# WD-Leong/CV-Lite-Object-Detection

Measured on AMD Instinct MI355X. Metric: training images/sec (whole node), FCOS-VOC 512x512 bs=16/GPU, higher is better.
Workload: dtype bf16; 1 GPU; FCOS ResNet-50-FPN train step (targets + fwd + loss + bwd + clip/SGD), 512x512, bs=16 per GPU; model=FCOS-ResNet50-FPN, global_batch=16, image_size=512, parallelism=dp1

## Files before the change

cv-lite-object-detection_amd/csrc/conv_common.h:

```cpp
#pragma once
#include "cvl_common.h"
#include "bn_acc.h"
#include <type_traits>
#include <vector>

typedef short s16x8 __attribute__((ext_vector_type(8)));
typedef short s16x4 __attribute__((ext_vector_type(4)));
typedef __bf16 bf16x8 __attribute__((ext_vector_type(8)));
typedef float f32x4 __attribute__((ext_vector_type(4)));

constexpr int kMaxSeg = CVL_CONV_MAX_SEG;

extern thread_local int g_cvl_conv_last_kernel;
extern thread_local int g_cvl_conv_last_ktile;

__device__ __forceinline__ int xcd_remap(int b, int nwg) {
  const int q = nwg / 8, r = nwg % 8, x = b % 8;
  return (x < r ? x * (q + 1) : r * (q + 1) + (x - r) * q) + b / 8;
}

template <int N>
__device__ __forceinline__ void wait_vm() {
  __builtin_amdgcn_s_waitcnt((N & 15) | ((N >> 4) << 14) | (7 << 4) | (15 << 8));
}

__device__ __forceinline__ s16x4 ds_tr16(unsigned addr) {
  s16x4 v;
  asm volatile("ds_read_b64_tr_b16 %0, %1" : "=v"(v) : "v"(addr));
  return v;
}
__device__ __forceinline__ void lgkm_wait() { asm volatile("s_waitcnt lgkmcnt(0)" ::: "memory"); }
__device__ __forceinline__ void tr_pin(s16x4& v) { asm volatile("" : "+v"(v)); }
__device__ __forceinline__ s16x8 tr_join(s16x4 l, s16x4 h) {
  return s16x8{l[0], l[1], l[2], l[3], h[0], h[1], h[2], h[3]};
}

__device__ __forceinline__ unsigned lds_addr(const void* p) {
  return (unsigned)(size_t)(const __attribute__((address_space(3))) void*)p;
}

struct ConvSeg {
  int Hr, Wr, Hs, Ws;
  long src_base, src_img, dst_base, dst_img;
  int m_start;
  int rows;
  const cvl_bf16* w;
  const float* bias;
// ... 51 lines not shown
int cvl_wgrad_reduce(const float* slab, float* dst0, float* dst1, long n4, int splits, int groups, float beta,
                     hipStream_t s);
int cvl_wgrad_defer_guard(const float* dst, hipStream_t s);
int cvl_wgrad_reduce_lanes(long elems4, int splits);

struct BnSumArgs {
  const cvl_bf16* z;
  const float* mr;
  const float* gamma;
  const float* beta;
  acc_u64* sums;
  float hi;
  const cvl_bf16* y;
  const uint8_t* bits;
};

enum { CVL_BSUM_NONE = 0, CVL_BSUM_Z = 1, CVL_BSUM_Y = 2, CVL_BSUM_BITS = 3 };
struct ConvCallOpts {
  bool bn_stats;
  int bsum;
  bool ymask;
  size_t workspace_bytes;
};

enum { CVL_PRE_NONE = 0, CVL_PRE_ZERO_GAPS = 1, CVL_PRE_S2DG3_PACK = 2 };

struct ConvPlan {
  int kernel;
  int bn, bk;
  bool dgrad;
  bool sw;
  bool wres;
  bool prio, acc, stamps;
  int stages;
  int bsum;
  bool ymask;
  int splits, ksteps_per_split;
  int grid;
  size_t workspace_bytes;
  int pre;
  size_t pack_bytes;
  int dbg;
  cvl_conv_desc desc;
  ConvArgs geo;
};

int conv_plan(const cvl_conv_desc* d, const ConvCallOpts& o, ConvPlan* p);
size_t conv_plan_workspace_bound(const cvl_conv_desc* d);
static inline void conv_plan_set_splits(ConvPlan* p, int nk, int want) {
  p->ksteps_per_split = (nk + want - 1) / want;
  p->splits = (nk + p->ksteps_per_split - 1) / p->ksteps_per_split;
}
static inline int conv_plan_ktile(const ConvPlan& p) { return p.kernel == CVL_CK_X32 || p.kernel == CVL_CK_P ? p.bk : 0; }

int launch_base(const ConvPlan& p, const ConvArgs& a, hipStream_t s);
int launch_l(const ConvPlan& p, const ConvArgs& a, hipStream_t s);
int launch_x(const ConvPlan& p, const ConvArgs& a, hipStream_t s);
int launch_h(const ConvPlan& p, const ConvArgs& a, hipStream_t s);
int launch_p(const ConvPlan& p, const ConvArgs& a, hipStream_t s);

bool cvl_conv_h_fits(const cvl_conv_desc* d, const ConvArgs& a, int* halo_px);
constexpr int kConvHWresCb = 2;
constexpr int kConvHStampWgs = 4096;
constexpr unsigned kConvBufRecords = 0x7fffffffu;

template <class F>
// ... 137 lines not shown
```

cv-lite-object-detection_amd/csrc/conv_dispatch.hip:

```cpp
#include "conv_common.h"

namespace {

constexpr int BM_BASE = 128, NT_BASE = 256;
constexpr int BM = 256;
constexpr int H_BN = 64, H_BK = 32;

int device_cus() {
  static const int n = cvl_device_cus();
  return n;
}

int pick_bn(int npad) { return npad % 128 == 0 ? 128 : (npad % 64 == 0 ? 64 : 32); }

int base_split_want(const ConvArgs& a) {
  if (a.nseg != 1) return 1;
  const int BN_ = pick_bn(a.Npad), BK_ = a.Cin % 64 == 0 ? 64 : 32;
  const int tiles = a.m_tiles * (a.Npad / BN_);
  const int nk = a.K / BK_;
  const int max_tiles = cvl_tune_int("CVL_KSPLIT_MAX_TILES", 192);
  const int target = cvl_tune_int("CVL_KSPLIT_TARGET", 384);
  const int min_nk = cvl_dispatch_int("ksplit_min_nk", 4);
  if (tiles >= max_tiles || nk < min_nk) return 1;
  int s = (target + tiles - 1) / tiles;
// ... 111 lines not shown
                 (a.dst_up != 1 && !by) || o.bn_stats || (a.seg[0].Hr * a.seg[0].Wr) % BM ||
                 (a.dst_up == 1 && a.seg[0].dst_img != (long)a.seg[0].Hr * a.seg[0].Wr) || a.Npad % 64))
    return false;
  if (d->mode == CVL_CONV_DGRAD && d->stride != 1) return false;
  const ConvSeg& q = a.seg[0];
  if (d->stride == 1 && (q.Hs != q.Hr || q.Ws != q.Wr)) return false;
  if (a.dst_f32 ? (a.n_store % 4 || a.ld_dst % 4 || a.dst_coff % 4) : !dst_chunks8(d)) return false;
  if (o.bn_stats && (a.dst_f32 || (q.Hr * q.Wr) % BM)) return false;
  return buffer_bounds_ok(a);
}

bool plan_p(const cvl_conv_desc* d, const ConvArgs& a, const ConvCallOpts& o, ConvPlan* p) {
  if (cvl_dispatch_flag("no_p") || !p_fits(d, a, o)) return false;
  if (o.bsum && cvl_tune_flag("CVL_CONV_P_NO_BSUM")) return false;
  const bool wide = a.K <= 256 || (a.Npad >= 2 * a.K && cvl_dispatch_int("p_wide128", 1));
  const int bn = wide && a.Npad % 128 == 0 ? 128 : (a.Npad % 64 == 0 ? 64 : 0);
  const int fbn = cvl_dispatch_int("p_bn", 0);
  const int use = o.bsum ? 64 : (fbn && a.Npad % fbn == 0 ? fbn : bn);
  if (!use) return false;
  const int ntiles = a.m_tiles * (a.Npad / use);
  const int ntn = a.Npad / use;
  const int wgs = cvl_dispatch_int("p_wgs", 256);
  int grid = cvl_tune_int("CVL_CONV_P_WGS", wgs > 256 ? 256 : (wgs < 1 ? 1 : wgs));
  if (grid >= ntiles) grid = ntiles;
  else grid -= grid % ntn;
  if (grid < 1) return false;
  p->kernel = CVL_CK_P;
  p->bn = use;
  p->bk = a.K % 64 == 0 && use != 256 && cvl_dispatch_int("p_k64", 1) ? 64 : 32;
  p->grid = grid;
  p->dbg = cvl_tune_int("CVL_P_ABLATE", 0);
  p->bsum = o.bsum;
  p->acc = a.beta != 0.f && !cvl_tune_flag("CVL_P_NO_ACC");
  return true;
}

bool plan_h(const cvl_conv_desc* d, const ConvArgs& a, const ConvCallOpts& o, size_t ws_bytes, ConvPlan* p) {
  int halo_px = 0;
  if (cvl_dispatch_flag("no_h") || !cvl_conv_h_fits(d, a, &halo_px)) return false;
  const bool stg3 = !cvl_dispatch_flag("h_no_3stage") && halo_px <= 512;
  const bool bs = o.bsum != CVL_BSUM_NONE;
  p->kernel = CVL_CK_H64;
  p->bk = H_BK;
  p->bsum = o.bsum;
  if (a.Npad == 32) {
    if (o.bn_stats || bs) return false;
    p->bn = 32;
    p->stages = stg3 ? 3 : 2;
    p->grid = a.m_tiles < device_cus() ? a.m_tiles : device_cus();
    return true;
  }
  const int tiles = a.m_tiles * (a.Npad / H_BN);
  const bool sw_ok = !d->dst_f32 && d->beta == 0.f && dst_chunks8(d) && !(o.bn_stats && bs) && tiles_in_images(a, bs);
  if (!cvl_dispatch_flag("h_no_n32") && a.Npad % H_BN == 0 && 2 * tiles <= device_cus() && sw_ok) {
    p->bn = 32;
    p->sw = true;
    p->stages = stg3 ? 3 : 2;
    p->grid = 2 * tiles;
    return true;
  }
  const int ncb = a.Cin / H_BK;
  int splits = 1;
  if (a.nseg == 1 && !bs && ws_bytes && d->n_store % 8 == 0 && d->dst_coff % 8 == 0 &&
      (d->dst_f32 || d->ld_dst % 8 == 0) && d->n_store / 8 <= 256) {
    splits = h_split_want(a);
    if (slab_bytes(a, splits) > ws_bytes) splits = 1;
// ... 205 lines not shown
```

cv-lite-object-detection_amd/csrc/conv_igemm.hip:

```cpp
#include "conv_common.h"

namespace {

constexpr int BM = 128;
constexpr int NT = 256;

template <int BK>
__device__ __forceinline__ int swz(int r) {
  return BK == 128 ? (r & 15) : (BK == 64 ? ((r >> 1) & 7) : ((r >> 2) & 3));
}

__device__ __forceinline__ s16x8 relu_bf16x8(s16x8 v) {
#pragma unroll
  for (int i = 0; i < 8; ++i) v[i] = v[i] < 0 ? (short)0 : v[i];
  return v;
}



template <int BN, int BK, bool DGRAD>
__global__ void __launch_bounds__(NT) conv_igemm_kernel(ConvArgs a) {
  constexpr int WM = BM / 2, WN = BN / 2;
  constexpr int TM = WM / 16, TN = WN / 16;
  constexpr int CPR = BK / 8;
// ... 438 lines not shown
  const void* ymask;
  void* workspace;
};

void fill_args(const ConvPlan& p, const ConvIo& io, ConvArgs* a) {
  *a = p.geo;
  a->src = reinterpret_cast<const cvl_bf16*>(io.src);
  a->dst = io.dst;
  a->stats = io.stats;
  if (p.bsum) {
    const BnSumArgs& b = *io.bsum;
    a->bz = b.z; a->bmr = b.mr; a->bga = b.gamma; a->bbe = b.beta; a->bsum = b.sums; a->bhi = b.hi;
    a->by = b.y;
    a->bbits = b.bits;
  }
  if (p.ymask) a->ymask = reinterpret_cast<const cvl_bf16*>(io.ymask);
  if (p.kernel == CVL_CK_X32) a->probe = reinterpret_cast<unsigned long long*>(cvl_probe_current(true));
  a->dbg = p.dbg;
  a->splits = p.splits;
  a->ksteps_per_split = p.ksteps_per_split;
  char* ws = reinterpret_cast<char*>(io.workspace);
  if (p.splits > 1) a->slab = reinterpret_cast<float*>(ws + p.pack_bytes);
  if (p.pre == CVL_PRE_S2DG3_PACK)
    for (int i = 0; i < kMaxSeg; ++i)
      a->seg[i].w = reinterpret_cast<const cvl_bf16*>(ws) + (size_t)(i < a->nseg ? i : 0) * a->Npad * a->K;
}

}

thread_local int g_cvl_conv_last_kernel = CVL_CK_NONE;
thread_local int g_cvl_conv_last_ktile = 0;

extern "C" int cvl_conv_igemm_last_kernel(void) { return g_cvl_conv_last_kernel; }
extern "C" int cvl_conv_igemm_last_ktile(void) { return g_cvl_conv_last_ktile; }

int launch_base(const ConvPlan& p, const ConvArgs& a, hipStream_t s) {
  if (p.bn == 128) launch_bn<128>(p, a, s);
  else if (p.bn == 64) launch_bn<64>(p, a, s);
  else launch_bn<32>(p, a, s);
  return cvl_launch_status();
}

namespace {
int conv_run(const ConvPlan& p, const cvl_conv_desc* d, const ConvIo& io, hipStream_t s) {
  int st = pre_pass(p, d, io.dst, io.workspace, s);
  if (st) return st;
  ConvArgs a;
  fill_args(p, io, &a);
  switch (p.kernel) {
    case CVL_CK_P: st = launch_p(p, a, s); break;
    case CVL_CK_X32: st = launch_x(p, a, s); break;
    case CVL_CK_H64: st = launch_h(p, a, s); break;
    case CVL_CK_L64: case CVL_CK_L128: case CVL_CK_L256: st = launch_l(p, a, s); break;
    default: st = launch_base(p, a, s); break;
  }
  g_cvl_conv_last_kernel = p.kernel;
  g_cvl_conv_last_ktile = conv_plan_ktile(p);
  if (st || p.splits <= 1) return st;
  return splitk_finish_launch(a, s);
}
}

extern "C" const char* cvl_conv_kernel_name(int code) {
  switch (code) {
    case CVL_CK_BASE: return "conv_igemm_kernel (128-row)";
    case CVL_CK_BASE_SPLITK: return "conv_igemm_kernel (128-row, split-K)";
    case CVL_CK_L64: return "conv_igemm_l_kernel<64> (256x64)";
    case CVL_CK_L128: return "conv_igemm_l_kernel<128> (256x128)";
    case CVL_CK_L256: return "conv_igemm_l_kernel<256> (256x256)";
    case CVL_CK_X256: return "conv_igemm_x_kernel (256x256, 4 phases per 64-deep K-tile)";
    case CVL_CK_X32: return "conv_igemm_x32_kernel (256x256, 5-slot ring of 32-deep K-tiles)";
    case CVL_CK_X32H: return "conv_igemm_x32h_kernel (256x256, 3x3 halo tile in LDS, 6-slot weight ring)";
    case CVL_CK_WG_SN: return "conv_wgrad_sn_kernel (Npad 32, taps on the dY side, chunk slabs)";
    case CVL_CK_WG_S: return "conv_wgrad_kernel (128-wide k tile)";
    case CVL_CK_WG_L128: return "conv_wgrad_l_kernel<128> (128x256)";
    case CVL_CK_WG_L256: return "conv_wgrad_l_kernel<256> (256x256)";
    case CVL_CK_WG_X: return "conv_wgrad_x_kernel (256x256, 5-slot ring of 32-row steps, grouped)";
    case CVL_CK_WG_H: return "conv_wgrad_h_kernel (64 ci x 64 co x 9 taps, 128-row halo steps)";
    case CVL_CK_H64: return "conv_igemm_h_kernel (256x64, 3x3 halo + 9-tap weight stage per channel block)";
    case CVL_CK_P: return "conv_igemm_p_kernel (persistent 1x1, K-tile stream across tiles)";
    default: return "none";
  }
}

int cvl_conv_f32(const cvl_conv_desc* d, const void* src, void* dst, acc_u64* bn_stats, hipStream_t s);
int cvl_relu_backward(const void* dy, const void* y, void* dx, long n, float beta, cvl_stream_t stream);

extern "C" size_t cvl_conv_igemm_workspace_size(const cvl_conv_desc* d) {
  if (!d) return 0;
  if (d->prec == CVL_PREC_F32) return 16;
// ... 141 lines not shown
```

cv-lite-object-detection_amd/csrc/conv_igemm_p.hip:

```cpp
#include "conv_common.h"

namespace {

constexpr int NT = 512, BM = 256;
constexpr unsigned kRecords = 0x7fffffffu;
constexpr unsigned kOOB = 0x80000000u;
constexpr int LDS_BYTES = 163840;

template <int BK>
__device__ __forceinline__ int swz(int r) { return (r >> 1) & (BK / 8 - 1); }

__device__ __forceinline__ void dma16(__amdgpu_buffer_rsrc_t r, const void* lds_dst, unsigned voff) {
  __builtin_amdgcn_raw_ptr_buffer_load_lds(r, (__attribute__((address_space(3))) void*)lds_dst, 16, (int)voff, 0,
                                           0, 0);
}

template <int BN, int BK>
struct PCfg {
  static constexpr int WGM = BN == 256 ? 2 : 4, WGN = 8 / WGM;
  static constexpr int WM = BM / WGM, WN = BN / WGN, TM = WM / 16, TN = WN / 16;
  static constexpr int SLOT_B = (BM + BN) * BK * 2;
  static constexpr int PR = 8 * 64 * 16 / (BK * 2);
  static constexpr int APW = BM / PR;
  static constexpr int BPW = BN >= PR ? BN / PR : 1;
  static constexpr int PW = APW + BPW;
  static constexpr int RED_B = WGM * BN * 2 * 4;
  static constexpr int DUMMY_B = BN < PR ? 4 * 1024 : 0;
  static constexpr int NS = (LDS_BYTES - RED_B - DUMMY_B) / SLOT_B;
  static constexpr int D = NS - 1;
  static_assert(D >= 2, "ring too short");
};

typedef __bf16 bf16x2 __attribute__((ext_vector_type(2)));
typedef float f32x2 __attribute__((ext_vector_type(2)));
typedef unsigned u32x4 __attribute__((ext_vector_type(4)));

__device__ __forceinline__ void wait_vm_atleast(int n) {
  if (n >= 63) wait_vm<63>();
  else if (n >= 48) wait_vm<48>();
  else if (n >= 36) wait_vm<36>();
  else if (n >= 30) wait_vm<30>();
  else if (n >= 24) wait_vm<24>();
  else if (n >= 21) wait_vm<21>();
  else if (n >= 18) wait_vm<18>();
  else if (n >= 15) wait_vm<15>();
  else if (n >= 12) wait_vm<12>();
  else if (n >= 9) wait_vm<9>();
  else if (n >= 6) wait_vm<6>();
  else if (n >= 3) wait_vm<3>();
  else wait_vm<0>();
}

__device__ __forceinline__ s16x8 gload16_untracked(const void* p) {
  s16x8 v;
  asm volatile("global_load_dwordx4 %0, %1, off" : "=v"(v) : "v"(p) : "memory");
  return v;
}
__device__ __forceinline__ void pin16(s16x8& v) { asm volatile("" : "+v"(v)); }
__device__ __forceinline__ unsigned gload1_untracked(const void* p) {
  unsigned v;
  asm volatile("global_load_ubyte %0, %1, off" : "=v"(v) : "v"(p) : "memory");
  return v;
}
__device__ __forceinline__ void pin1(unsigned& v) { asm volatile("" : "+v"(v)); }

template <int BN, int BK, bool RELU, bool F32, int BS = 0, bool ACC = false>
__global__ void __launch_bounds__(NT) conv_igemm_p_kernel(ConvArgs a, int ntiles) {
  using C = PCfg<BN, BK>;
  constexpr int TM = C::TM, TN = C::TN, NS = C::NS, D = C::D;
  __shared__ __attribute__((aligned(16))) char lds[C::NS * C::SLOT_B + C::RED_B + C::DUMMY_B];
  float* red = reinterpret_cast<float*>(lds + NS * C::SLOT_B);
  char* dummy = lds + NS * C::SLOT_B + C::RED_B;

  const int tid = threadIdx.x;
  const int wave = __builtin_amdgcn_readfirstlane(tid >> 6), lane = tid & 63;
  const ConvSeg& S = a.seg[0];
  const int HWr = S.Hr * S.Wr;
  const int ntn = a.Npad / BN;
  const int nk = a.K / BK;
  const int G = gridDim.x;
  const int L = xcd_remap(blockIdx.x, G);
  const int nmc = G / ntn;
  const int mchunk = (a.m_tiles + nmc - 1) / nmc;
  const int mt0 = (L / ntn) * mchunk;
  const int my_tiles = max(0, min(mchunk, a.m_tiles - mt0));
  const int total = my_tiles * nk;
  const bool dense_src = a.stride == 1 && S.Hs == S.Hr && S.Ws == S.Wr && S.src_img == (long)HWr;
  const int Cin2 = a.Cin * 2;
  const int K2 = a.K * 2;

  constexpr int LPR = BK / 8, PR = C::PR, WR = PR / 8;
  const int prow = wave * WR + lane / LPR, ch = lane % LPR;
  const unsigned chs = (unsigned)((ch ^ swz<BK>(prow)) * 16);
  const __amdgpu_buffer_rsrc_t rsA = __builtin_amdgcn_make_buffer_rsrc((void*)a.src, (short)0, (int)kRecords, 0x00020000);
  const __amdgpu_buffer_rsrc_t rsB = __builtin_amdgcn_make_buffer_rsrc((void*)S.w, (short)0, (int)kRecords, 0x00020000);

  int ik = 0, it = 0, islot = 0;
  unsigned ia[C::APW], ib[C::BPW];
  const int n0 = (L % ntn) * BN;
  auto set_issue_tile = [&](int k) {
    const int m0 = (mt0 + k) * BM;
#pragma unroll
    for (int p = 0; p < C::APW; ++p) {
// ... 56 lines not shown
  for (int i = 0; i < TM; ++i)
#pragma unroll
    for (int j = 0; j < TN; ++j) acc[i][j] = f32x4{0.f, 0.f, 0.f, 0.f};

  float bcol[TN][4];
#pragma unroll
  for (int j = 0; j < TN; ++j)
#pragma unroll
    for (int e = 0; e < 4; ++e) {
      const int n = n0 + wn * C::WN + j * 16 + 4 * lg + e;
      bcol[j][e] = (S.bias && n < a.n_store) ? S.bias[n] : 0.f;
    }
  constexpr int NJP = BS ? TN / 2 : 1;
  const int lgo = ((lg & 1) ? 16 : 0) + ((lg & 2) ? 8 : 0);
  float bga[NJP][8], bbe[NJP][8], bm[NJP][8], brs[NJP][8], bs1[NJP][8], bs2[NJP][8];
  int bimg = -1;
  if (BS) {
#pragma unroll
    for (int jp = 0; jp < NJP; ++jp)
#pragma unroll
      for (int u = 0; u < 8; ++u) {
        const int c = n0 + wn * C::WN + jp * 32 + lgo + u;
        bga[jp][u] = a.bga[c];
        bbe[jp][u] = a.bbe[c];
        bs1[jp][u] = 0.f;
        bs2[jp][u] = 0.f;
      }
  }
  wait_vm<0>();
  s16x8 zv[BS ? TM : 1][NJP];
  s16x8 yv[BS == 2 ? TM : 1][BS == 2 ? NJP : 1];
  unsigned bv[BS == 3 ? TM : 1][BS == 3 ? NJP : 1];
  s16x8 ov[ACC ? TM : 1][ACC ? TN / 2 : 1];

  float ss1[TN][4], ss2[TN][4];
#pragma unroll
  for (int j = 0; j < TN; ++j)
#pragma unroll
    for (int e = 0; e < 4; ++e) { ss1[j][e] = 0.f; ss2[j][e] = 0.f; }
  auto row16_sum = [](float v) {
    v += __int_as_float(__builtin_amdgcn_mov_dpp(__float_as_int(v), 0xB1, 0xF, 0xF, false));
    v += __int_as_float(__builtin_amdgcn_mov_dpp(__float_as_int(v), 0x4E, 0xF, 0xF, false));
    v += __int_as_float(__builtin_amdgcn_mov_dpp(__float_as_int(v), 0x141, 0xF, 0xF, false));
    v += __int_as_float(__builtin_amdgcn_mov_dpp(__float_as_int(v), 0x140, 0xF, 0xF, false));
    return v;
  };
  auto flush_stats = [&](int img) {
#pragma unroll
    for (int j = 0; j < TN; ++j)
#pragma unroll
      for (int e = 0; e < 4; ++e) {
        const float s1 = row16_sum(ss1[j][e]), s2 = row16_sum(ss2[j][e]);
        ss1[j][e] = 0.f;
        ss2[j][e] = 0.f;
        if (lr == 0) {
          const int c = wn * C::WN + j * 16 + 4 * lg + e;
          red[(wm * BN + c) * 2] = s1;
          red[(wm * BN + c) * 2 + 1] = s2;
        }
      }
    __syncthreads();
    if (tid < BN && n0 + tid < a.n_store) {
      float t1 = 0.f, t2 = 0.f;
#pragma unroll
      for (int w = 0; w < C::WGM; ++w) { t1 += red[(w * BN + tid) * 2]; t2 += red[(w * BN + tid) * 2 + 1]; }
      acc_u64* st = a.stats + acc_idx((long)img * a.n_store + n0 + tid, 0, a.acc_slots);
// ... 1 lines not shown
      acc_add(st + a.acc_slots, t2, a.acc_slots);
    }
  };

  auto flush_bsum = [&](int img) {
#pragma unroll
    for (int jp = 0; jp < NJP; ++jp)
#pragma unroll
      for (int u = 0; u < 8; ++u) {
        const float t1 = row16_sum(bs1[jp][u]), t2 = row16_sum(bs2[jp][u]);
        bs1[jp][u] = 0.f;
        bs2[jp][u] = 0.f;
        if (lr == 0) {
          const int c = wn * C::WN + jp * 32 + lgo + u;
          red[(wm * BN + c) * 2] = t1;
          red[(wm * BN + c) * 2 + 1] = t2;
        }
      }
    __syncthreads();
    if (tid < BN && n0 + tid < a.n_store) {
      float t1 = 0.f, t2 = 0.f;
#pragma unroll
      for (int w = 0; w < C::WGM; ++w) { t1 += red[(w * BN + tid) * 2]; t2 += red[(w * BN + tid) * 2 + 1]; }
      acc_u64* st = a.bsum + acc_idx((long)img * a.n_store + n0 + tid, 0, a.acc_slots);
      acc_add(st, t1, a.acc_slots);
      acc_add(st + a.acc_slots, t2, a.acc_slots);
    }
  };

  auto epilogue = [&](int k) {
    const int m0 = (mt0 + k) * BM;
    const bool dense_dst = a.dst_up == 1 && S.dst_img == (long)HWr;
    const bool do_stats = a.stats && !(a.dbg & 1);
    if (ACC) {
      wait_vm_atleast(C::PW * (nk - 1));
#pragma unroll
      for (int i = 0; i < TM; ++i)
#pragma unroll
        for (int jp = 0; jp < TN / 2; ++jp) pin16(ov[i][jp]);
    }
    if (BS) {
      wait_vm_atleast(C::PW * (nk - 1));
#pragma unroll
      for (int i = 0; i < TM; ++i)
#pragma unroll
        for (int jp = 0; jp < NJP; ++jp) {
          pin16(zv[i][jp]);
          if (BS == 2) pin16(yv[i][jp]);
          if (BS == 3) pin1(bv[i][jp]);
        }
      const int img = m0 / HWr;
      if (img != bimg) {
        bimg = img;
#pragma unroll
        for (int jp = 0; jp < NJP; ++jp)
#pragma unroll
          for (int u = 0; u < 8; ++u) {
            const long bc = (long)img * a.n_store + n0 + wn * C::WN + jp * 32 + lgo + u;
            bm[jp][u] = a.bmr[bc * 2];
            brs[jp][u] = a.bmr[bc * 2 + 1];
          }
      }
    }
#pragma unroll
    for (int i = 0; i < TM; ++i) {
      const int ml = m0 + wm * C::WM + i * 16 + lr;
      const bool row_ok = ml < S.rows && !(a.dbg & 2);
      long drow;
      if (dense_dst || !row_ok) {
        drow = S.dst_base + ml;
      } else {
        const int img = ml / HWr, q = ml - img * HWr;
        drow = conv_dst_row(a, S, img, q);
      }
      if (F32) {
#pragma unroll
        for (int j = 0; j < TN; ++j) {
          f32x4 v;
#pragma unroll
          for (int e = 0; e < 4; ++e) {
            v[e] = acc[i][j][e] + bcol[j][e];
            if (RELU) v[e] = fmaxf(v[e], 0.f);
          }
          const int n = n0 + wn * C::WN + j * 16 + 4 * lg;
          if (!row_ok || n >= a.n_store) continue;
          f32x4* pd = reinterpret_cast<f32x4*>(reinterpret_cast<float*>(a.dst) + drow * a.ld_dst + a.dst_coff + n);
          if (a.beta != 0.f) v += a.beta * *pd;
          *pd = v;
        }
        continue;
      }
#pragma unroll
      for (int j = 0; j < TN; j += 2) {
        unsigned pk[2][2];
#pragma unroll
        for (int jj = 0; jj < 2; ++jj)
#pragma unroll
          for (int h = 0; h < 2; ++h) {
            float v0 = acc[i][j + jj][2 * h] + bcol[j + jj][2 * h];
            float v1 = acc[i][j + jj][2 * h + 1] + bcol[j + jj][2 * h + 1];
            if (RELU) { v0 = fmaxf(v0, 0.f); v1 = fmaxf(v1, 0.f); }
            const unsigned u = __builtin_bit_cast(unsigned, __builtin_convertvector((f32x2){v0, v1}, bf16x2));
            pk[jj][h] = u;
            if (do_stats) {
              const float r0 = __uint_as_float(u << 16), r1 = __uint_as_float(u & 0xffff0000u);
              ss1[j + jj][2 * h] += r0;
              ss2[j + jj][2 * h] = __builtin_fmaf(r0, r0, ss2[j + jj][2 * h]);
              ss1[j + jj][2 * h + 1] += r1;
              ss2[j + jj][2 * h + 1] = __builtin_fmaf(r1, r1, ss2[j + jj][2 * h + 1]);
            }
          }
#pragma unroll
        for (int h = 0; h < 2; ++h) {
          const auto sw = __builtin_amdgcn_permlane16_swap(pk[0][h], pk[1][h], false, false);
          pk[0][h] = sw[0];
          pk[1][h] = sw[1];
        }
        const int n = n0 + wn * C::WN + j * 16 + ((lg & 1) ? 16 : 0) + ((lg & 2) ? 8 : 0);
        if (!row_ok || n >= a.n_store) continue;
        s16x8* pd = reinterpret_cast<s16x8*>(reinterpret_cast<cvl_bf16*>(a.dst) + drow * a.ld_dst + a.dst_coff + n);
        s16x8 o = __builtin_bit_cast(s16x8, (u32x4){pk[0][0], pk[0][1], pk[1][0], pk[1][1]});
        if (ACC) {
          const s16x8 old = ov[i][j / 2];
#pragma unroll
          for (int u = 0; u < 8; ++u)
            o[u] = (short)f32_to_bf16(bf16_to_f32((cvl_bf16)o[u]) + a.beta * bf16_to_f32((cvl_bf16)old[u]));
        } else if (a.beta != 0.f) {
          const s16x8 old = *pd;
#pragma unroll
          for (int u = 0; u < 8; ++u)
            o[u] = (short)f32_to_bf16(bf16_to_f32((cvl_bf16)o[u]) + a.beta * bf16_to_f32((cvl_bf16)old[u]));
        }
        if (BS) {
          const s16x8 zz = zv[i][j / 2];
#pragma unroll
          for (int u = 0; u < 8; ++u) {
            const float zf = bf16_to_f32((cvl_bf16)zz[u]);
            const float xh = (zf - bm[j / 2][u]) * brs[j / 2][u];
            bool on;
            if (BS == 2) {
              on = bf16_to_f32((cvl_bf16)yv[i][j / 2][u]) > 0.f;
            } else if (BS == 3) {
              on = (bv[i][j / 2] >> u) & 1u;
            } else {
              const float af = __builtin_fmaf(bga[j / 2][u], xh, bbe[j / 2][u]);
              on = af > 0.f && af < a.bhi;
            }
            const float gv = on ? bf16_to_f32((cvl_bf16)o[u]) : 0.f;
            bs1[j / 2][u] += gv;
            bs2[j / 2][u] = __builtin_fmaf(gv, xh, bs2[j / 2][u]);
          }
        }
        *pd = o;
      }
    }
    if (do_stats) {
      const int img = m0 / HWr;
      if (k == my_tiles - 1 || (m0 + BM) / HWr != img) flush_stats(img);
    }
    if (BS) {
      const int img = m0 / HWr;
      if (k == my_tiles - 1 || (m0 + BM) / HWr != img) flush_bsum(img);
    }
#pragma unroll
    for (int i = 0; i < TM; ++i)
#pragma unroll
      for (int j = 0; j < TN; ++j) acc[i][j] = f32x4{0.f, 0.f, 0.f, 0.f};
  };

  unsigned long long* stamp = ((a.dbg & 8) && tid == 0) ? reinterpret_cast<unsigned long long*>(a.dst) + blockIdx.x * 4 : nullptr;
  if (stamp) stamp[0] = wall_clock64();
#pragma unroll
  for (int d = 0; d < D; ++d) issue();
  int rslot = 0, ck = 0, ct = 0;
  for (int g = 0; g < total; ++g) {
    wait_vm<(D - 1) * C::PW>();
    __builtin_amdgcn_s_barrier();
    asm volatile("" ::: "memory");
    issue();
    if (ACC && ck == 0) {
      const int m0 = (mt0 + ct) * BM;
      const bool dense_dst = a.dst_up == 1 && S.dst_img == (long)HWr;
#pragma unroll
      for (int i = 0; i < TM; ++i) {
        const int ml = m0 + wm * C::WM + i * 16 + lr;
        long drow = S.dst_base;
        if (ml < S.rows) {
          if (dense_dst) {
            drow = S.dst_base + ml;
          } else {
            const int img = ml / HWr, q = ml - img * HWr;
            drow = conv_dst_row(a, S, img, q);
          }
        }
#pragma unroll
        for (int jp = 0; jp < TN / 2; ++jp) {
          int n = n0 + wn * C::WN + jp * 32 + lgo;
          if (n >= a.n_store) n = 0;
          ov[i][jp] = gload16_untracked(reinterpret_cast<const cvl_bf16*>(a.dst) + drow * a.ld_dst + a.dst_coff + n);
        }
      }
    }
    if (BS && ck == 0) {
      const int m0 = (mt0 + ct) * BM;
      const bool dense_dst = a.dst_up == 1 && S.dst_img == (long)HWr;
#pragma unroll
      for (int i = 0; i < TM; ++i)
#pragma unroll
        for (int jp = 0; jp < NJP; ++jp) {
          const int ml = m0 + wm * C::WM + i * 16 + lr;
          long row = S.dst_base + ml;
          if (!dense_dst && ml < S.rows) {
            const int img = ml / HWr, q = ml - img * HWr;
            row = conv_dst_row(a, S, img, q);
          }
          zv[i][jp] = gload16_untracked(a.bz + row * a.ld_dst + a.dst_coff + n0 + wn * C::WN + jp * 32 + lgo);
          if (BS == 2)
            yv[i][jp] = gload16_untracked(a.by + row * a.ld_dst + a.dst_coff + n0 + wn * C::WN + jp * 32 + lgo);
          if (BS == 3)
            bv[i][jp] = gload1_untracked(a.bbits + ((row * a.ld_dst + a.dst_coff + n0 + wn * C::WN + jp * 32 + lgo) >> 3));
        }
    }
    const char* sl = lds + rslot * C::SLOT_B;
#pragma unroll
    for (int kh = 0; kh < BK / 32; ++kh) {
      s16x8 fa[TM], fb[TN];
#pragma unroll
      for (int i = 0; i < TM; ++i) fa[i] = *reinterpret_cast<const s16x8*>(sl + (fao[i] ^ (unsigned)(kh * 64)));
#pragma unroll
      for (int j = 0; j < TN; ++j) fb[j] = *reinterpret_cast<const s16x8*>(sl + (fbo[j] ^ (unsigned)(kh * 64)));
#pragma unroll
      for (int i = 0; i < TM; ++i)
#pragma unroll
        for (int j = 0; j < TN; ++j)
          acc[i][j] = __builtin_amdgcn_mfma_f32_16x16x32_bf16(__builtin_bit_cast(bf16x8, fb[j]),
                                                               __builtin_bit_cast(bf16x8, fa[i]), acc[i][j], 0, 0, 0);
    }
    rslot = rslot == NS - 1 ? 0 : rslot + 1;
    if (++ck == nk) {
      ck = 0;
      epilogue(ct);
      ++ct;
    }
  }
  wait_vm<0>();
  if (stamp) { stamp[1] = wall_clock64(); stamp[2] = total; }
}

template <int BN_, int BK_, bool ACC_>
void p_launch(const ConvPlan& p, const ConvArgs& a, hipStream_t s) {
  const dim3 grid(p.grid);
  const int ntiles = a.m_tiles * (a.Npad / p.bn);
  if (p.bsum == CVL_BSUM_BITS) {
    hipLaunchKernelGGL((conv_igemm_p_kernel<64, BK_, false, false, 3, true>), grid, dim3(NT), 0, s, a, ntiles);
  } else if (p.bsum == CVL_BSUM_Y) {
    hipLaunchKernelGGL((conv_igemm_p_kernel<64, BK_, false, false, 2, true>), grid, dim3(NT), 0, s, a, ntiles);
  } else if (p.bsum) {
    hipLaunchKernelGGL((conv_igemm_p_kernel<64, BK_, false, false, 1>), grid, dim3(NT), 0, s, a, ntiles);
  } else if (a.dst_f32) {
    with_bool(a.relu_out != 0, [&](auto RELU) {
      hipLaunchKernelGGL((conv_igemm_p_kernel<BN_, BK_, decltype(RELU)::value, true>), grid, dim3(NT), 0, s, a, ntiles);
    });
  } else if (a.relu_out) {
    hipLaunchKernelGGL((conv_igemm_p_kernel<BN_, BK_, true, false>), grid, dim3(NT), 0, s, a, ntiles);
  } else if (p.acc) {
    hipLaunchKernelGGL((conv_igemm_p_kernel<BN_, BK_, false, false, false, ACC_>), grid, dim3(NT), 0, s, a, ntiles);
  } else {
    hipLaunchKernelGGL((conv_igemm_p_kernel<BN_, BK_, false, false>), grid, dim3(NT), 0, s, a, ntiles);
  }
}

}

int launch_p(const ConvPlan& p, const ConvArgs& a, hipStream_t s) {
  if (p.bn == 256) p_launch<256, 32, false>(p, a, s);
  else if (p.bn == 128 && p.bk == 64) p_launch<128, 64, true>(p, a, s);
  else if (p.bn == 128) p_launch<128, 32, true>(p, a, s);
  else if (p.bk == 64) p_launch<64, 64, true>(p, a, s);
  else p_launch<64, 32, true>(p, a, s);
  return cvl_launch_status();
}
```

cv-lite-object-detection_amd/cvlite/_lib.py:

```python
import ctypes
import os

import torch

_HERE = os.path.dirname(os.path.abspath(__file__))
LIB_PATH = os.environ.get("CVL_LIB") or os.path.join(_HERE, "libcvlite_hip.so")


def dispatch(key, default=0):
    for tok in os.environ.get("CVL_DISPATCH", "").split(","):
        k, _, v = tok.strip().partition("=")
        if k == key:
            return int(v) if v else 1
    return default

c_int, c_float, c_size_t, c_void_p = ctypes.c_int, ctypes.c_float, ctypes.c_size_t, ctypes.c_void_p
P = c_void_p

SIGNATURES = {
    "cvl_version": (c_int, []),
    "cvl_fcos_assign": (c_int, [P, P, P, c_int, c_int, c_int, c_int, c_int, P, P, P, P, P]),
    "cvl_fcos_loss_workspace_size": (c_size_t, [c_int, c_int]),
    "cvl_fcos_loss": (c_int, [P, c_int, P, c_int, P, c_int, c_int, c_int, c_int, c_float, P,
                              P, c_int, c_int, P, c_int, c_int, P, c_size_t, P]),
    "cvl_fcos_loss_ex": (c_int, [P, c_int, P, c_int, P, c_int, c_int, c_int, c_int, c_float, c_float, c_float,
                                 c_float, P, P, c_int, c_int, P, c_int, c_int, P, c_size_t, P]),
    "cvl_fcos_decode": (c_int, [P, c_int, c_int, c_int, ctypes.c_double, P, P]),
    "cvl_fcos_v1_decode": (c_int, [P, c_int, c_int, c_int, c_float, c_float, P, P]),
    "cvl_conv_igemm_workspace_size": (c_size_t, [P]),
    "cvl_conv_igemm": (c_int, [P, P, P, P, P, c_size_t, P]),
    "cvl_conv_igemm_relu_mask": (c_int, [P, P, P, P, P, c_size_t, P]),
    "cvl_conv_igemm_last_kernel": (c_int, []),
    "cvl_conv_igemm_last_ktile": (c_int, []),
    "cvl_conv_igemm_plan": (c_int, [P, c_int, c_size_t, P, P]),
    "cvl_conv_igemm_plan_grid": (c_int, [P, c_int, c_int, c_size_t, P, P, P, P]),
    "cvl_conv_kernel_name": (ctypes.c_char_p, [c_int]),
    "cvl_conv_igemm_plan_bnsum": (c_int, [P, c_int, c_size_t, P, P, P]),
    "cvl_conv_igemm_dgrad_bnsum_res_bits": (c_int, [P, P, P, P, P, P, P, P, P, P, P, P, P, ctypes.c_size_t, P]),
    "cvl_bn_finalize_apply_bits": (c_int, [P, P, P, P, P, P, P, P, P, P, c_int, c_int, c_int, c_int, c_float,
                                           c_float, P]),
    "cvl_bn_finalize_apply_bnres_bits": (c_int, [P, P, P, P, P, P, P, P, P, P, P, P, P, P, c_float, c_float, P, P,
                                                 c_int, c_int, c_int, c_int, c_float, c_float, P]),
    "cvl_bn_backward_bits": (c_int, [P, P, P, P, P, P, c_size_t, P, P, P, P, c_float, P, c_int, c_int, c_int, P]),
    "cvl_bn_backward_res_sums_bits": (c_int, [P, P, P, P, P, P, P, P, P, P, c_float, P, c_int, c_int, c_int, P]),
    "cvl_bn_backward_res_sums_sc_bits": (c_int, [P, P, P, P, P, P, P, P, P, P, c_float, P, P, P, P, c_size_t, P,
                                                 c_int, c_int, c_int, P]),
    "cvl_bn_backward_sc_bits": (c_int, [P, P, P, P, P, P, c_size_t, P, P, P, P, c_float, P, P, P, P, c_int, c_int,
                                        c_int, P]),
    "cvl_centernet_peak_decode_workspace_size": (ctypes.c_size_t, [c_int, c_int, c_int, c_int]),
    "cvl_centernet_peak_decode": (c_int, [P, c_int, c_int, c_int, c_int, c_int, c_float, c_float, c_int, P, P, P,
                                          ctypes.c_size_t, P]),
    "cvl_conv_igemm_dgrad_bnsum": (c_int, [P, P, P, P, P, P, P, c_float, P, P, P, ctypes.c_size_t, P]),
    "cvl_bn_backward_relu_sums": (c_int, [P, P, P, P, P, P, P, P, P, c_float, P, c_float, c_int, c_int, c_int, P]),
    "cvl_conv_igemm_dgrad_bnsum_res": (c_int, [P, P, P, P, P, P, P, P, P, P, P, ctypes.c_size_t, P]),
    "cvl_bn_backward_res_sums": (c_int, [P, P, P, P, P, P, P, P, P, P, c_float, P, c_int, c_int, c_int, P]),
    "cvl_bn_backward_res_sums_sc_workspace_size": (c_size_t, [c_int, c_int, c_int]),
    "cvl_bn_backward_res_sums_sc": (c_int, [P, P, P, P, P, P, P, P, P, P, c_float, P, P, P, P, c_size_t, P, c_int,
                                            c_int, c_int, P]),
    "cvl_bn_backward_sums": (c_int, [P, P, P, P, P, P, P, P, c_float, P, c_int, c_int, c_int, P]),
    "cvl_bn_backward_sc_workspace_size": (c_size_t, [c_int, c_int, c_int]),
    "cvl_bn_backward_sc": (c_int, [P, P, P, P, P, P, c_size_t, P, P, P, P, c_float, P, P, P, P, c_int, c_int, c_int, P]),
    "cvl_probe_arm": (c_int, [P]),
    "cvl_probe_clock_hz": (ctypes.c_double, []),
    "cvl_conv_wgrad_workspace_size": (c_size_t, [P]),
    "cvl_conv_wgrad": (c_int, [P, P, P, P, c_float, P, c_size_t, P]),
    "cvl_conv_wgrad_grouped_workspace_size": (c_size_t, [P, c_int]),
# ... 112 lines not shown
                                P, P, P, c_size_t, P]),
    "cvl_jpeg_info": (c_int, [P, c_size_t, P]),
    "cvl_jpeg_entropy_decode": (c_int, [P, c_size_t, P, c_size_t, P]),
    "cvl_jpeg_batch_sizes": (c_int, [P, c_int, P, P]),
    "cvl_jpeg_decode_batch": (c_int, [P, P, c_int, P, P, c_size_t, P, c_size_t, P, P]),
    "cvl_bn_apply_f32": (c_int, [P, P, P, P, P, P, c_int, c_int, c_int, c_int, P]),
    "cvl_bn_finalize_apply_f32": (c_int, [P, P, P, P, P, P, P, P, P, c_int, c_int, c_int, c_int, c_float, c_float,
                                          P]),
    "cvl_bn_backward_f32_workspace_size": (c_size_t, [c_int, c_int]),
    "cvl_bn_backward_f32": (c_int, [P, P, P, P, P, P, P, c_size_t, P, P, P, P, c_float, P, c_float, c_int, c_int,
                                    c_int, P]),
    "cvl_maxpool3x3s2_f32": (c_int, [P, P, P, c_int, c_int, c_int, c_int, P]),
    "cvl_maxpool3x3s2_backward_f32": (c_int, [P, P, P, c_int, c_int, c_int, c_int, P]),
    "cvl_upsample2x_add_f32": (c_int, [P, P, P, c_int, c_int, c_int, c_int, P]),
    "cvl_upsample2x_backward_f32": (c_int, [P, P, c_int, c_int, c_int, c_int, c_float, P]),
    "cvl_relu_backward_f32": (c_int, [P, P, P, ctypes.c_long, c_float, P]),
    "cvl_add_f32": (c_int, [P, P, P, ctypes.c_long, P]),
    "cvl_bias_grad_multi_f32": (c_int, [P, c_int, P]),
    "cvl_retina_loss_f32": (c_int, [P, c_int, P, c_int, P, c_int, P, c_int, c_int, P, c_float, P, P, c_int, P, c_int,
                                    P, P]),
}


class CvlError(RuntimeError):
    pass


_lib = None


NEWER = {"cvl_conv_igemm_last_ktile", "cvl_conv_igemm_plan", "cvl_conv_igemm_plan_bnsum", "cvl_conv_igemm_plan_grid",
         "cvl_conv_igemm_dgrad_bnsum_res_bits", "cvl_bn_finalize_apply_bits", "cvl_bn_finalize_apply_bnres_bits",
         "cvl_bn_backward_bits", "cvl_bn_backward_res_sums_bits", "cvl_bn_backward_res_sums_sc_bits",
         "cvl_bn_backward_sc_bits", "cvl_conv_wgrad_plan", "cvl_conv_wgrad_batch_plan"}


def load():
    global _lib
    if _lib is None:
        if not os.path.exists(LIB_PATH):
            raise CvlError("cvlite native library not built (%s): run __graft_entry__.build() or "
                           "make -C cv-lite-object-detection_amd/csrc" % LIB_PATH)
        lib = ctypes.CDLL(LIB_PATH)
        for name, (res, args) in SIGNATURES.items():
            if name in NEWER and os.environ.get("CVL_LIB") and not hasattr(lib, name):
                continue
            fn = getattr(lib, name)
            fn.restype = res
            fn.argtypes = args
        _lib = lib
        if os.environ.get("CVL_BN_EXACT", "0") == "1":
            lib.cvl_bn_set_exact(1)
    return _lib


def call(name, *args):
    st = getattr(load(), name)(*args)
    if st != 0:
        if st >= 1000:
            raise CvlError("%s failed: hipError %d" % (name, st - 1000))
        raise CvlError("%s: invalid argument (status %d)" % (name, st))
    return True


def ptr(t):
    return None if t is None else c_void_p(t.data_ptr())

# ... 14 lines not shown
```

include/cvlite.h:

```cpp
#ifndef CVLITE_H_
#define CVLITE_H_

#include <stddef.h>
#include <stdint.h>

#ifdef __cplusplus
extern "C" {
#endif

typedef void* cvl_stream_t;

enum { CVL_OK = 0, CVL_EINVAL = 1, CVL_EHIP = 1000 };

int cvl_version(void);

int cvl_fcos_assign(const float* boxes, const int32_t* nbox, const float* img_dim, int B, int n_max,
                    int pad_h, int pad_w, int num_classes, const int32_t* strides ,
                    const float* size_bounds , float* targets, int32_t* num_targets,
                    cvl_stream_t stream);

size_t cvl_fcos_loss_workspace_size(int B, int P);
int cvl_fcos_loss(const float* reg_pred, int ld_reg, const float* cls_pred, int ld_cls,
                  const float* targets, int B, int P, int num_classes, int reg_type,
                  float grad_scale, float* losses, void* d_reg, int ld_dreg, int dreg_dtype,
// ... 34 lines not shown
  const float* bias;
} cvl_conv_seg;

typedef struct {
  int mode;
  int B;
  int Cin;
  int KH, KW, stride, pad_t, pad_l;
  int Npad;
  int n_store;
  int ld_dst, dst_coff;
  int dst_f32;
  int relu_out;
  int relu_in;
  float beta;
  int nseg;
  cvl_conv_seg seg[CVL_CONV_MAX_SEG];
  int prec;
} cvl_conv_desc;
enum { CVL_PREC_BF16 = 0, CVL_PREC_F32 = 1 };

size_t cvl_conv_igemm_workspace_size(const cvl_conv_desc* d);
int cvl_conv_igemm(const cvl_conv_desc* d, const void* src, void* dst, uint64_t* bn_stats,
                   void* workspace, size_t workspace_bytes, cvl_stream_t stream);
int cvl_conv_igemm_relu_mask(const cvl_conv_desc* d, const void* src, void* dst, const void* y, void* workspace,
                             size_t workspace_bytes, cvl_stream_t stream);

enum { CVL_CK_NONE = 0, CVL_CK_BASE = 1, CVL_CK_BASE_SPLITK = 2, CVL_CK_L64 = 3, CVL_CK_L128 = 4,
       CVL_CK_L256 = 5, CVL_CK_X256 = 6, CVL_CK_X32 = 7,
       CVL_CK_WG_S = 8, CVL_CK_WG_L128 = 9, CVL_CK_WG_L256 = 10, CVL_CK_WG_X = 11, CVL_CK_X32H = 12, CVL_CK_WG_SN = 13,
       CVL_CK_H64 = 14, CVL_CK_WG_H = 15, CVL_CK_P = 16 };
int cvl_conv_igemm_last_kernel(void);
int cvl_conv_igemm_last_ktile(void);
int cvl_conv_igemm_plan(const cvl_conv_desc* d, int with_bn_stats, size_t workspace_bytes, int32_t* kernel,
                        int32_t* ktile);
int cvl_conv_igemm_plan_grid(const cvl_conv_desc* d, int with_bn_stats, int bsum_offer, size_t workspace_bytes,
                             int32_t* kernel, int32_t* ktile, int32_t* grid, int32_t* ntile);
const char* cvl_conv_kernel_name(int code);

int cvl_probe_arm(uint64_t* slot);
double cvl_probe_clock_hz(void);

size_t cvl_conv_wgrad_workspace_size(const cvl_conv_desc* d);
int cvl_conv_wgrad(const cvl_conv_desc* d, const void* x, const void* dy, float* dw, float beta,
                   void* workspace, size_t workspace_bytes, cvl_stream_t stream);

int cvl_wgrad_defer(int on, cvl_stream_t stream);
int cvl_wgrad_flush(cvl_stream_t stream);
size_t cvl_conv_wgrad_grouped_workspace_size(const cvl_conv_desc* d, int ngroups);
int cvl_conv_wgrad_grouped(const cvl_conv_desc* d, int ngroups, const void* x, const void* dy, float* const* dw,
                           float beta, void* workspace, size_t workspace_bytes, cvl_stream_t stream);

size_t cvl_conv_wgrad_batch_workspace_size(const cvl_conv_desc* const* d, int n);
int cvl_conv_wgrad_batch(const cvl_conv_desc* const* d, int n, const void* const* x, const void* const* dy,
                         float* const* dw, float beta, void* workspace, size_t workspace_bytes, cvl_stream_t stream);

int cvl_conv_wgrad_plan(const cvl_conv_desc* d, int ngroups, int32_t* kernel, int32_t* tile, int32_t* nsplit,
                        size_t* workspace);
int cvl_conv_wgrad_batch_plan(const cvl_conv_desc* const* d, int n, int32_t* kernel_of, int32_t* launch_of,
                              int32_t* nsplit_of);

int cvl_pack_conv_weights(const float* w_hwio, int KH, int KW, int Cin, int Cout, int Cin_k, int Npad,
                          void* w_fwd, int Cin_pad, int Cout_pad, void* w_dgrad, cvl_stream_t stream);

typedef struct {
  const float* w;
// ... 362 lines not shown
```

Before: 1420 images/s.

## Stage residual and bitmap epilogue loads through LDS in the persistent conv kernel

Adds a staged variant of the persistent (P) conv kernel for the 64x64 bitmap-residual accumulate form with short K. Instead of holding the old-output and z residual values in registers and waiting on them before the epilogue, each wave DMAs them into a dedicated LDS staging area and prefetches the next tile's rows right after finishing the current tile. It uses computed vmcnt wait counts. The ring shrinks to two slots to make LDS room, which reduces mainloop pipelining depth, and the wait-count arithmetic is fragile. Host query helpers for the wait counts and the staging flag are added.

```diff
diff --git a/cv-lite-object-detection_amd/csrc/conv_common.h b/cv-lite-object-detection_amd/csrc/conv_common.h
--- a/cv-lite-object-detection_amd/csrc/conv_common.h
+++ b/cv-lite-object-detection_amd/csrc/conv_common.h
@@ -13,6 +13,23 @@
 
 extern thread_local int g_cvl_conv_last_kernel;
 extern thread_local int g_cvl_conv_last_ktile;
+
+extern thread_local int g_cvl_conv_last_pstage;
+
+constexpr int kPStageRB = 4, kPStageSG = 3, kPStageST = 1, kPStagePW = 5;
+__host__ __device__ constexpr int p_stage_ring_younger(int t, int k) {
+  return k ? 0 : kPStageRB * (kPStageSG + (t ? kPStageST : 0));
+}
+__host__ __device__ constexpr int p_stage_rb_younger(int nk, int t, int T, int i) {
+  return (kPStageRB - 1 - i) * (kPStageSG + (t ? kPStageST : 0)) + nk * kPStagePW +
+         i * (kPStageST + (t + 1 < T ? kPStageSG : 0));
+}
+__host__ __device__ constexpr int p_vm_bucket(int n) {
+  constexpr int b[12] = {63, 48, 36, 30, 24, 21, 18, 15, 12, 9, 6, 3};
+  for (int i = 0; i < 12; ++i)
+    if (n >= b[i]) return b[i];
+  return 0;
+}
 
 __device__ __forceinline__ int xcd_remap(int b, int nwg) {
   const int q = nwg / 8, r = nwg % 8, x = b % 8;
@@ -130,6 +147,7 @@
   bool sw;
   bool wres;
   bool prio, acc, stamps;
+  bool pstage;
   int stages;
   int bsum;
   bool ymask;
diff --git a/cv-lite-object-detection_amd/csrc/conv_dispatch.hip b/cv-lite-object-detection_amd/csrc/conv_dispatch.hip
--- a/cv-lite-object-detection_amd/csrc/conv_dispatch.hip
+++ b/cv-lite-object-detection_amd/csrc/conv_dispatch.hip
@@ -167,6 +167,11 @@
   p->dbg = cvl_tune_int("CVL_P_ABLATE", 0);
   p->bsum = o.bsum;
   p->acc = a.beta != 0.f && !cvl_tune_flag("CVL_P_NO_ACC");
+  const ConvSeg& q = a.seg[0];
+  const long dst_bytes = (q.dst_base + (long)a.B * q.dst_img) * a.ld_dst * 2;
+  p->pstage = o.bsum == CVL_BSUM_BITS && p->acc && !p->dbg && use == 64 && p->bk == 64 &&
+              a.K / 64 <= cvl_dispatch_int("p_stage", 2) && a.n_store == a.Npad && q.rows % BM == 0 &&
+              dst_bytes < (long)kConvBufRecords - 65536;
   return true;
 }
 
diff --git a/cv-lite-object-detection_amd/csrc/conv_igemm.hip b/cv-lite-object-detection_amd/csrc/conv_igemm.hip
--- a/cv-lite-object-detection_amd/csrc/conv_igemm.hip
+++ b/cv-lite-object-detection_amd/csrc/conv_igemm.hip
@@ -494,7 +494,13 @@
 thread_local int g_cvl_conv_last_ktile = 0;
 
 extern "C" int cvl_conv_igemm_last_kernel(void) { return g_cvl_conv_last_kernel; }
+thread_local int g_cvl_conv_last_pstage = 0;
 extern "C" int cvl_conv_igemm_last_ktile(void) { return g_cvl_conv_last_ktile; }
+extern "C" int cvl_conv_igemm_last_pstage(void) { return g_cvl_conv_last_pstage; }
+extern "C" int cvl_p_stage_wait_count(int ring, int nk, int t, int tiles, int i) {
+  return ring ? p_stage_ring_younger(t, i) : p_stage_rb_younger(nk, t, tiles, i);
+}
+extern "C" int cvl_p_stage_wait_bucket(int n) { return p_vm_bucket(n); }
 
 int launch_base(const ConvPlan& p, const ConvArgs& a, hipStream_t s) {
   if (p.bn == 128) launch_bn<128>(p, a, s);
@@ -518,6 +524,7 @@
   }
   g_cvl_conv_last_kernel = p.kernel;
   g_cvl_conv_last_ktile = conv_plan_ktile(p);
+  if (p.kernel == CVL_CK_P) g_cvl_conv_last_pstage = p.pstage ? 1 : 0;
   if (st || p.splits <= 1) return st;
   return splitk_finish_launch(a, s);
 }
diff --git a/cv-lite-object-detection_amd/csrc/conv_igemm_p.hip b/cv-lite-object-detection_amd/csrc/conv_igemm_p.hip
--- a/cv-lite-object-detection_amd/csrc/conv_igemm_p.hip
+++ b/cv-lite-object-detection_amd/csrc/conv_igemm_p.hip
@@ -15,7 +15,7 @@
                                            0, 0);
 }
 
-template <int BN, int BK>
+template <int BN, int BK, bool STG = false>
 struct PCfg {
   static constexpr int WGM = BN == 256 ? 2 : 4, WGN = 8 / WGM;
   static constexpr int WM = BM / WGM, WN = BN / WGN, TM = WM / 16, TN = WN / 16;
@@ -26,9 +26,12 @@
   static constexpr int PW = APW + BPW;
   static constexpr int RED_B = WGM * BN * 2 * 4;
   static constexpr int DUMMY_B = BN < PR ? 4 * 1024 : 0;
-  static constexpr int NS = (LDS_BYTES - RED_B - DUMMY_B) / SLOT_B;
+  static constexpr int STG_SLOT_B = 2048;
+  static constexpr int STG_B = STG ? 8 * (BM / WGM / 16) * STG_SLOT_B : 0;
+  static constexpr int NS = STG ? 2 : (LDS_BYTES - RED_B - DUMMY_B) / SLOT_B;
   static constexpr int D = NS - 1;
-  static_assert(D >= 2, "ring too short");
+  static_assert(D >= (STG ? 1 : 2), "ring too short");
+  static_assert(NS * SLOT_B + RED_B + DUMMY_B + STG_B <= LDS_BYTES, "LDS");
 };
 
 typedef __bf16 bf16x2 __attribute__((ext_vector_type(2)));
@@ -64,11 +67,13 @@
 }
 __device__ __forceinline__ void pin1(unsigned& v) { asm volatile("" : "+v"(v)); }
 
-template <int BN, int BK, bool RELU, bool F32, int BS = 0, bool ACC = false>
+template <int BN, int BK, bool RELU, bool F32, int BS = 0, bool ACC = false, bool STG = false>
 __global__ void __launch_bounds__(NT) conv_igemm_p_kernel(ConvArgs a, int ntiles) {
-  using C = PCfg<BN, BK>;
+  using C = PCfg<BN, BK, STG>;
   constexpr int TM = C::TM, TN = C::TN, NS = C::NS, D = C::D;
-  __shared__ __attribute__((aligned(16))) char lds[C::NS * C::SLOT_B + C::RED_B + C::DUMMY_B];
+  static_assert(!STG || (BN == 64 && BK == 64 && BS == 3 && ACC), "staged form: the bitmap residual form, 64 x 64");
+  static_assert(!STG || (TM == kPStageRB && TN == 2 && C::PW == kPStagePW), "p_stage_*_younger (conv_common.h)");
+  __shared__ __attribute__((aligned(16))) char lds[C::NS * C::SLOT_B + C::RED_B + C::DUMMY_B + C::STG_B];
   float* red = reinterpret_cast<float*>(lds + NS * C::SLOT_B);
   char* dummy = lds + NS * C::SLOT_B + C::RED_B;
 
@@ -191,6 +196,27 @@
   s16x8 yv[BS == 2 ? TM : 1][BS == 2 ? NJP : 1];
   unsigned bv[BS == 3 ? TM : 1][BS == 3 ? NJP : 1];
   s16x8 ov[ACC ? TM : 1][ACC ? TN / 2 : 1];
+  char* stg = lds + NS * C::SLOT_B + C::RED_B + C::DUMMY_B + wave * (TM * C::STG_SLOT_B);
+  const __amdgpu_buffer_rsrc_t rsO = __builtin_amdgcn_make_buffer_rsrc((void*)a.dst, (short)0, (int)kRecords, 0x00020000);
+  const __amdgpu_buffer_rsrc_t rsZ = __builtin_amdgcn_make_buffer_rsrc((void*)a.bz, (short)0, (int)kRecords, 0x00020000);
+  unsigned soff[STG ? TM : 1];
+  auto stage_issue = [&](int k, int i) {
+    if (k > 0 && a.dst_up == 1 && S.dst_img == (long)HWr) {
+      soff[STG ? i : 0] += (unsigned)(BM * a.ld_dst * 2);
+    } else {
+      const int ml = (mt0 + k) * BM + wm * C::WM + i * 16 + lr;
+      long row = S.dst_base + ml;
+      if (!(a.dst_up == 1 && S.dst_img == (long)HWr)) {
+        const int img = ml / HWr, q = ml - img * HWr;
+        row = conv_dst_row(a, S, img, q);
+      }
+      soff[STG ? i : 0] = (unsigned)((row * a.ld_dst + a.dst_coff + n0 + wn * C::WN + lgo) * 2);
+    }
+    const unsigned off = soff[STG ? i : 0];
+    dma16(rsO, stg + i * C::STG_SLOT_B, off);
+    dma16(rsZ, stg + i * C::STG_SLOT_B + 1024, off);
+    bv[BS == 3 ? i : 0][0] = gload1_untracked(a.bbits + (off >> 4));
+  };
 
   float ss1[TN][4], ss2[TN][4];
 #pragma unroll
@@ -258,7 +284,7 @@
     const int m0 = (mt0 + k) * BM;
     const bool dense_dst = a.dst_up == 1 && S.dst_img == (long)HWr;
     const bool do_stats = a.stats && !(a.dbg & 1);
-    if (ACC) {
+    if (ACC && !STG) {
       wait_vm_atleast(C::PW * (nk - 1));
 #pragma unroll
       for (int i = 0; i < TM; ++i)
@@ -266,15 +292,17 @@
         for (int jp = 0; jp < TN / 2; ++jp) pin16(ov[i][jp]);
     }
     if (BS) {
-      wait_vm_atleast(C::PW * (nk - 1));
-#pragma unroll
-      for (int i = 0; i < TM; ++i)
-#pragma unroll
-        for (int jp = 0; jp < NJP; ++jp) {
-          pin16(zv[i][jp]);
-          if (BS == 2) pin16(yv[i][jp]);
-          if (BS == 3) pin1(bv[i][jp]);
-        }
+      if (!STG) {
+        wait_vm_atleast(C::PW * (nk - 1));
+#pragma unroll
+        for (int i = 0; i < TM; ++i)
+#pragma unroll
+          for (int jp = 0; jp < NJP; ++jp) {
+            pin16(zv[i][jp]);
+            if (BS == 2) pin16(yv[i][jp]);
+            if (BS == 3) pin1(bv[i][jp]);
+          }
+      }
       const int img = m0 / HWr;
       if (img != bimg) {
         bimg = img;
@@ -315,6 +343,14 @@
           *pd = v;
         }
         continue;
+      }
+      s16x8 sov = {}, szv = {};
+      if (STG) {
+        wait_vm_atleast(p_stage_rb_younger(nk, k, my_tiles, i));
+        asm volatile("" ::: "memory");
+        sov = *reinterpret_cast<const s16x8*>(stg + i * C::STG_SLOT_B + lane * 16);
+        szv = *reinterpret_cast<const s16x8*>(stg + i * C::STG_SLOT_B + 1024 + lane * 16);
+        pin1(bv[BS == 3 ? i : 0][0]);
       }
 #pragma unroll
       for (int j = 0; j < TN; j += 2) {
@@ -343,11 +379,12 @@
           pk[1][h] = sw[1];
         }
         const int n = n0 + wn * C::WN + j * 16 + ((lg & 1) ? 16 : 0) + ((lg & 2) ? 8 : 0);
-        if (!row_ok || n >= a.n_store) continue;
-        s16x8* pd = reinterpret_cast<s16x8*>(reinterpret_cast<cvl_bf16*>(a.dst) + drow * a.ld_dst + a.dst_coff + n);
+        if (!STG && (!row_ok || n >= a.n_store)) continue;
+        s16x8* pd = STG ? reinterpret_cast<s16x8*>(reinterpret_cast<char*>(a.dst) + soff[STG ? i : 0])
+                        : reinterpret_cast<s16x8*>(reinterpret_cast<cvl_bf16*>(a.dst) + drow * a.ld_dst + a.dst_coff + n);
         s16x8 o = __builtin_bit_cast(s16x8, (u32x4){pk[0][0], pk[0][1], pk[1][0], pk[1][1]});
         if (ACC) {
-          const s16x8 old = ov[i][j / 2];
+          const s16x8 old = STG ? sov : ov[i][j / 2];
 #pragma unroll
           for (int u = 0; u < 8; ++u)
             o[u] = (short)f32_to_bf16(bf16_to_f32((cvl_bf16)o[u]) + a.beta * bf16_to_f32((cvl_bf16)old[u]));
@@ -358,7 +395,7 @@
             o[u] = (short)f32_to_bf16(bf16_to_f32((cvl_bf16)o[u]) + a.beta * bf16_to_f32((cvl_bf16)old[u]));
         }
         if (BS) {
-          const s16x8 zz = zv[i][j / 2];
+          const s16x8 zz = STG ? szv : zv[i][j / 2];
 #pragma unroll
           for (int u = 0; u < 8; ++u) {
             const float zf = bf16_to_f32((cvl_bf16)zz[u]);
@@ -379,6 +416,7 @@
         }
         *pd = o;
       }
+      if (STG && k + 1 < my_tiles) stage_issue(k + 1, i);
     }
     if (do_stats) {
       const int img = m0 / HWr;
@@ -398,13 +436,18 @@
   if (stamp) stamp[0] = wall_clock64();
 #pragma unroll
   for (int d = 0; d < D; ++d) issue();
+  if (STG && my_tiles > 0) {
+#pragma unroll
+    for (int i = 0; i < TM; ++i) stage_issue(0, i);
+  }
   int rslot = 0, ck = 0, ct = 0;
   for (int g = 0; g < total; ++g) {
-    wait_vm<(D - 1) * C::PW>();
+    if (STG) wait_vm_atleast(p_stage_ring_younger(ct, ck));
+    else wait_vm<(D - 1) * C::PW>();
     __builtin_amdgcn_s_barrier();
     asm volatile("" ::: "memory");
     issue();
-    if (ACC && ck == 0) {
+    if (ACC && !STG && ck == 0) {
       const int m0 = (mt0 + ct) * BM;
       const bool dense_dst = a.dst_up == 1 && S.dst_img == (long)HWr;
 #pragma unroll
@@ -427,7 +470,7 @@
         }
       }
     }
-    if (BS && ck == 0) {
+    if (BS && !STG && ck == 0) {
       const int m0 = (mt0 + ct) * BM;
       const bool dense_dst = a.dst_up == 1 && S.dst_img == (long)HWr;
 #pragma unroll
@@ -477,7 +520,10 @@
 void p_launch(const ConvPlan& p, const ConvArgs& a, hipStream_t s) {
   const dim3 grid(p.grid);
   const int ntiles = a.m_tiles * (a.Npad / p.bn);
-  if (p.bsum == CVL_BSUM_BITS) {
+  if (p.bsum == CVL_BSUM_BITS && p.pstage) {
+    if constexpr (BK_ == 64)
+      hipLaunchKernelGGL((conv_igemm_p_kernel<64, 64, false, false, 3, true, true>), grid, dim3(NT), 0, s, a, ntiles);
+  } else if (p.bsum == CVL_BSUM_BITS) {
     hipLaunchKernelGGL((conv_igemm_p_kernel<64, BK_, false, false, 3, true>), grid, dim3(NT), 0, s, a, ntiles);
   } else if (p.bsum == CVL_BSUM_Y) {
     hipLaunchKernelGGL((conv_igemm_p_kernel<64, BK_, false, false, 2, true>), grid, dim3(NT), 0, s, a, ntiles);
diff --git a/cv-lite-object-detection_amd/cvlite/_lib.py b/cv-lite-object-detection_amd/cvlite/_lib.py
--- a/cv-lite-object-detection_amd/cvlite/_lib.py
+++ b/cv-lite-object-detection_amd/cvlite/_lib.py
@@ -32,6 +32,9 @@
     "cvl_conv_igemm_relu_mask": (c_int, [P, P, P, P, P, c_size_t, P]),
     "cvl_conv_igemm_last_kernel": (c_int, []),
     "cvl_conv_igemm_last_ktile": (c_int, []),
+    "cvl_conv_igemm_last_pstage": (c_int, []),
+    "cvl_p_stage_wait_count": (c_int, [c_int, c_int, c_int, c_int, c_int]),
+    "cvl_p_stage_wait_bucket": (c_int, [c_int]),
     "cvl_conv_igemm_plan": (c_int, [P, c_int, c_size_t, P, P]),
     "cvl_conv_igemm_plan_grid": (c_int, [P, c_int, c_int, c_size_t, P, P, P, P]),
     "cvl_conv_kernel_name": (ctypes.c_char_p, [c_int]),
@@ -210,7 +213,8 @@
 NEWER = {"cvl_conv_igemm_last_ktile", "cvl_conv_igemm_plan", "cvl_conv_igemm_plan_bnsum", "cvl_conv_igemm_plan_grid",
          "cvl_conv_igemm_dgrad_bnsum_res_bits", "cvl_bn_finalize_apply_bits", "cvl_bn_finalize_apply_bnres_bits",
          "cvl_bn_backward_bits", "cvl_bn_backward_res_sums_bits", "cvl_bn_backward_res_sums_sc_bits",
-         "cvl_bn_backward_sc_bits", "cvl_conv_wgrad_plan", "cvl_conv_wgrad_batch_plan"}
+         "cvl_bn_backward_sc_bits", "cvl_conv_wgrad_plan", "cvl_conv_wgrad_batch_plan",
+         "cvl_conv_igemm_last_pstage", "cvl_p_stage_wait_count", "cvl_p_stage_wait_bucket"}
 
 
 def load():
diff --git a/include/cvlite.h b/include/cvlite.h
--- a/include/cvlite.h
+++ b/include/cvlite.h
@@ -90,6 +90,9 @@
        CVL_CK_H64 = 14, CVL_CK_WG_H = 15, CVL_CK_P = 16 };
 int cvl_conv_igemm_last_kernel(void);
 int cvl_conv_igemm_last_ktile(void);
+int cvl_conv_igemm_last_pstage(void);
+int cvl_p_stage_wait_count(int ring, int nk, int t, int tiles, int i);
+int cvl_p_stage_wait_bucket(int n);
 int cvl_conv_igemm_plan(const cvl_conv_desc* d, int with_bn_stats, size_t workspace_bytes, int32_t* kernel,
                         int32_t* ktile);
 int cvl_conv_igemm_plan_grid(const cvl_conv_desc* d, int with_bn_stats, int bsum_offer, size_t workspace_bytes,
```

Result: no change. 1426 images/s (median of 6 runs) (+0.4%).
